# nv-tlabs/ChronoEdit

Hardware: AMD Instinct MI355X
Metric: denoising-steps/sec (higher is better)
Workload: dtype bf16

## Files before the change

chronoedit_amd/csrc/ce_attn.hip:

```cpp
#include <cstdlib>

#include "ce_common.h"

namespace {

constexpr int HD = 128;
constexpr int QW = 32;
constexpr int KVB = 64;
constexpr int K_TILE_BYTES = KVB * HD * 2;
constexpr int VT_TILE_BYTES = HD * KVB * 2;
constexpr int BUF_BYTES = K_TILE_BYTES + VT_TILE_BYTES;
constexpr int OST_ROW = HD * 2 + 16;
constexpr int smem_bytes(int nwave, bool two_seg) {
  const int stage = nwave * QW * OST_ROW;
  return two_seg ? 2 * BUF_BYTES + stage : (stage > 2 * BUF_BYTES ? stage : 2 * BUF_BYTES);
}
constexpr float NEG_BIG = -1.0e30f;

__device__ __forceinline__ int vt_swz(int dv) {
  return ((((dv >> 2) & 7) << 1) | (((dv >> 1) ^ (dv >> 5)) & 1)) ^ (((dv >> 6) & 1) << 1);
}

struct KVSeg {
  const bf16* k;
// ... 223 lines not shown
#pragma unroll
  for (int i = 0; i < 8; ++i) {
    const int c = lane + 64 * i;
    const int rl = c >> 4, cc = c & 15;
    const int q = q0 + rl;
    if (q < Nq) {
      const u32x4 v = *reinterpret_cast<const u32x4*>(smem + (TWO_SEG ? 2 * BUF_BYTES : 0) + (size_t)(wave * QW + rl) * OST_ROW + cc * 16);
      *reinterpret_cast<u32x4*>(O + (size_t)q * ldo + hoff + cc * 8) = v;
    }
  }
}


#define CE_EPOCH_BARRIER()                          \
  asm volatile("s_waitcnt lgkmcnt(0)" ::: "memory"); \
  __builtin_amdgcn_s_barrier()
constexpr int PK_ROW = HD * 2 + 16;
constexpr int PV_ROW = KVB * 2 + 16;
constexpr int PK_TILE = KVB * PK_ROW;
constexpr int PV_TILE = HD * PV_ROW;
typedef __attribute__((ext_vector_type(4))) unsigned pp_u4;
typedef __attribute__((ext_vector_type(2))) unsigned pp_u2;

constexpr int K_GRP = 1088;
typedef __attribute__((address_space(3))) void lds_void;
#ifdef CE_DIAGNOSTICS
__device__ unsigned long long g_sp_exact_hits = 0ull;
#endif
constexpr float SP_SPEC_THR = 1024.0f;
constexpr int SP_V0 = 2 * PK_TILE;
constexpr int SP_TILE_BYTES = 2 * PK_TILE + 3 * PV_TILE;
constexpr int sp_smem_bytes(bool two_seg) { return two_seg ? SP_TILE_BYTES + 8 * QW * OST_ROW : SP_TILE_BYTES; }

template <bool TWO_SEG, bool VT = false, bool QOUT = false>
__global__ __launch_bounds__(512, 2) void attn_fwd_sp_kernel(const bf16* __restrict__ Q_, bf16* __restrict__ O_, KVSeg seg0_,
                                                              KVSeg seg1_, int Nq, int H, int ldq, int ldo, int nqb,
                                                              float scale_log2e, int batch, BlkRows blk) {
  extern __shared__ __attribute__((aligned(16))) unsigned char smem[];
  constexpr int NWAVE = 8, QB = QW * NWAVE;
  const int tid = threadIdx.x, lane = tid & 63;
  const int wave = __builtin_amdgcn_readfirstlane(tid >> 6);
  const int l31 = lane & 31, hh = lane >> 5;
  for (int item = blockIdx.x; item < nqb * H * batch; item += gridDim.x) {
  const bf16* Q = Q_;
  bf16* O = O_;
  KVSeg seg0 = seg0_, seg1 = seg1_;

  int head, qb, bz;
  {
    const int nqb_full = Nq / QB;
    if ((H & 7) == 0) {
      const int xcd = item & 7, local = item >> 3, hx_n = H >> 3;
      const int full = batch * hx_n * nqb_full;
      if (local < full) {
        bz = local / (hx_n * nqb_full);
        const int r = local % (hx_n * nqb_full);
        head = xcd + 8 * (r / nqb_full);
        qb = r % nqb_full;
      } else {
        const int l2 = local - full;
        bz = l2 / hx_n;
        head = xcd + 8 * (l2 % hx_n);
        qb = nqb_full;
      }
    } else {
      bz = item / (nqb * H);
      const int r = item % (nqb * H);
      head = r / nqb;
      qb = r % nqb;
    }
  }
  {
    if (VT && blk.rows > 0) {
      Q += (size_t)bz * blk.rows * ldq;
      O += (size_t)bz * blk.rows * ldo;
      seg0.k += (size_t)bz * blk.rows * seg0.ldk;
      seg0.v += (size_t)bz * blk.vt_cols;
    } else {
      Q += (size_t)bz * Nq * ldq;
      O += (size_t)bz * Nq * ldo;
      seg0.k += (size_t)bz * seg0.len * seg0.ldk;
      seg0.v += VT ? (size_t)bz * (TWO_SEG ? blk.vt_cols : seg0.len) : (size_t)bz * seg0.len * seg0.ldv;
    }
    if (TWO_SEG) {
      seg1.k += (size_t)bz * seg1.len * seg1.ldk;
      seg1.v += VT ? (size_t)bz * blk.stride : (size_t)bz * seg1.len * seg1.ldv;
    }
  }
  const int q0 = qb * QB + wave * QW;
  const int hoff = head * HD;
  const bool active = q0 < Nq;
  const int q0row = (VT && blk.rows > 0) ? (q0 / blk.rows) * blk.stride + q0 % blk.rows : q0;

  bf16x8 qf[8];
  {
    const bf16* qrow = Q + (size_t)(q0 + l31 < Nq ? q0row + l31 : 0) * ldq + hoff + 8 * hh;
#pragma unroll
    for (int ks = 0; ks < 8; ++ks) qf[ks] = *reinterpret_cast<const bf16x8*>(qrow + 16 * ks);
  }
  auto scale_q = [&]() __attribute__((always_inline)) {
#pragma unroll
  for (int ks = 0; ks < 8; ++ks) {
    const u32x4 w = __builtin_bit_cast(u32x4, qf[ks]);
    u32x4 o;
#pragma unroll
    for (int i = 0; i < 4; ++i) o[i] = pack_bf16(bf16lo(w[i]) * scale_log2e, bf16hi(w[i]) * scale_log2e);
    qf[ks] = __builtin_bit_cast(bf16x8, o);
  }
#pragma unroll
  for (int ks = 0; ks < 8; ++ks) asm volatile("" : "+v"(qf[ks]));

  };
  const int v_dvq = (tid & 1) | (((tid >> 4) & 15) << 1), v_kvq = ((tid >> 1) & 7) | (((tid >> 8) & 1) << 3);
  const int v_chunk = (v_kvq & ~3) | ((v_kvq & 1) << 1) | ((v_kvq >> 1) & 1);
  unsigned char* ost = smem + (TWO_SEG ? SP_TILE_BYTES : 0) + (size_t)(wave * QW + l31) * OST_ROW;
  const int k_w = l31 & 3;
  const unsigned char* k_rd = smem + (l31 >> 2) * K_GRP + k_w * 256 + ((hh ^ (k_w & 1)) << 4);
  const int k_eo[2] = {(k_w >> 1) << 5, ((k_w >> 1) ^ 1) << 5};
  const unsigned char* v_rd = smem + SP_V0 + l31 * PV_ROW + hh * 16;
  int vt_off[4];
#pragma unroll
  for (int s4 = 0; s4 < 4; ++s4) {
    const int x = (l31 >> 1) & 7;
    vt_off[s4] = l31 * 128 + ((2 * (s4 ^ (x >> 1)) + (hh ^ (x & 1))) << 4);
  }
  unsigned char* v_wr = smem + SP_V0 + (4 * v_dvq) * PV_ROW + v_chunk * 8;

#pragma unroll
  for (int sidx = 0; sidx < (TWO_SEG ? 2 : 1); ++sidx) {
    const KVSeg sg = sidx == 0 ? seg0 : seg1;
    const int ntiles = (sg.len + KVB - 1) / KVB;
    const int k_rows_span = (VT && blk.rows > 0) ? ((sg.len - 1) / blk.rows) * blk.stride + blk.rows : sg.len;
    const auto k_rsrc = __builtin_amdgcn_make_buffer_rsrc((void*)(sg.k + hoff), 0, (k_rows_span - 1) * sg.ldk * 2 + HD * 2, 0x00020000);
    const auto v_rsrc = VT ? __builtin_amdgcn_make_buffer_rsrc((void*)(sg.v + (size_t)hoff * sg.ldv), 0, ((HD - 1) * sg.ldv + ntiles * KVB) * 2, 0x00020000)
                           : __builtin_amdgcn_make_buffer_rsrc((void*)(sg.v + hoff), 0, (sg.len - 1) * sg.ldv * 2 + HD * 2, 0x00020000);
    int v_voff[4];
#pragma unroll
    for (int i = 0; i < 4; ++i) v_voff[i] = (4 * v_kvq + i) * sg.ldv * 2 + v_dvq * 8;
    const int k_tile_bytes = KVB * sg.ldk * 2, v_tile_bytes = KVB * sg.ldv * 2;

    f32x16 oacc[4];
#pragma unroll
    for (int m = 0; m < 4; ++m)
#pragma unroll
      for (int r = 0; r < 16; ++r) oacc[m][r] = 0.f;
    float l_run = 0.f, alpha_prev = 1.0f, mc = 0.f;
    f32x16 cinit;
#pragma unroll
// ... 25 lines not shown
#pragma unroll
      for (int i = 0; i < 4; ++i) vreg[i] = __builtin_amdgcn_raw_buffer_load_b64(v_rsrc, v_voff[i], so, 0);
    };
    auto store_v_part = [&](int buf, int j) {
      const int w = j >> 1;
      uint32_t lo, hi;
      if ((j & 1) == 0) {
        lo = (vreg[0][w] & 0xffffu) | (vreg[1][w] << 16);
        hi = (vreg[2][w] & 0xffffu) | (vreg[3][w] << 16);
      } else {
        lo = (vreg[0][w] >> 16) | (vreg[1][w] & 0xffff0000u);
        hi = (vreg[2][w] >> 16) | (vreg[3][w] & 0xffff0000u);
      }
      pp_u2 val = {lo, hi};
      *reinterpret_cast<pp_u2*>(v_wr + buf * PV_TILE + j * PV_ROW) = val;
    };
    auto store_v = [&](int buf) {
#pragma unroll
      for (int j = 0; j < 4; ++j) {
        const int w = j >> 1;
        uint32_t lo, hi;
        if ((j & 1) == 0) {
          lo = (vreg[0][w] & 0xffffu) | (vreg[1][w] << 16);
          hi = (vreg[2][w] & 0xffffu) | (vreg[3][w] << 16);
        } else {
          lo = (vreg[0][w] >> 16) | (vreg[1][w] & 0xffff0000u);
          hi = (vreg[2][w] >> 16) | (vreg[3][w] & 0xffff0000u);
        }
        pp_u2 val = {lo, hi};
        *reinterpret_cast<pp_u2*>(v_wr + buf * PV_TILE + j * PV_ROW) = val;
      }
    };

    if (TWO_SEG && sidx == 1) { CE_EPOCH_BARRIER(); }
    dma_k(0, 0, 0);
    dma_k(0, 0, 1);
    __builtin_amdgcn_sched_barrier(0);
    if (VT) {
      dma_v(0, 0, 0);
      dma_v(0, 0, 1);
    } else {
      load_v(0);
    }
    {
      const pp_u4 z = {0u, 0u, 0u, 0u};
      for (int i = tid; i < PV_TILE / 16; i += NWAVE * 64) *reinterpret_cast<pp_u4*>(smem + SP_V0 + 2 * PV_TILE + i * 16) = z;
    }
    if (!VT) {
      store_v(0);
      asm volatile("s_waitcnt vmcnt(0)" ::: "memory");
      load_v(1);
    }
    if (sidx == 0) scale_q();

#define CE_SP_KWAIT()                                          \
  do {                                                         \
    if (VT) asm volatile("s_waitcnt vmcnt(2)" ::: "memory");   \
    else asm volatile("s_waitcnt vmcnt(4)" ::: "memory");      \
  } while (0)
    int vb_prev = 2, vb_cur = 0;

    for (int t = 0; !active && t < ntiles; ++t) {
      CE_SP_KWAIT();
      CE_EPOCH_BARRIER();
      const int vb_next = 3 - vb_prev - vb_cur;
      dma_k(t + 1, (t + 1) & 1, 0);
      dma_k(t + 1, (t + 1) & 1, 1);
      __builtin_amdgcn_sched_barrier(0);
      if (VT) {
        dma_v(t + 1, vb_next, 0);
        dma_v(t + 1, vb_next, 1);
      } else {
        store_v(vb_next);
        load_v(t + 2);
      }
      vb_prev = vb_cur;
      vb_cur = vb_next;
    }
    for (int t = 0; active && t < ntiles; ++t) {
      CE_SP_KWAIT();
      CE_EPOCH_BARRIER();
      const int vb_next = 3 - vb_prev - vb_cur;
      const unsigned char* kb = k_rd + (t & 1) * PK_TILE;
      const unsigned char* vb = v_rd + vb_prev * PV_TILE;
      const unsigned char* vtb = smem + SP_V0 + vb_prev * PV_TILE;

      const f32x16 zero16 = {0.f, 0.f, 0.f, 0.f, 0.f, 0.f, 0.f, 0.f, 0.f, 0.f, 0.f, 0.f, 0.f, 0.f, 0.f, 0.f};
      f32x16 st[2];
      {
        constexpr int RING = VT ? 4 : 6;
        bf16x8 kf[RING];
#define CE_LDK(i) (*reinterpret_cast<const bf16x8*>(kb + k_eo[((i) >> 1) & 1] + ((i) & 1) * 8 * K_GRP + ((i) >> 2) * 64))
#pragma unroll
// ... 107 lines not shown
          const bf16x8 kfr = *reinterpret_cast<const bf16x8*>(kb + k_eo[(i >> 1) & 1] + (i & 1) * 8 * K_GRP + (i >> 2) * 64);
          st[i & 1] = __builtin_amdgcn_mfma_f32_32x32x16_bf16(kfr, qf[i >> 1], i < 2 ? zero16 : st[i & 1], 0, 0, 0);
        }
#pragma unroll
        for (int f = 0; f < 2; ++f)
#pragma unroll
          for (int r = 0; r < 16; ++r) st[f][r] -= mc;
        mask_tail();
        rebase();
        psum = 0.f;
#pragma unroll
        for (int j = 0; j < 16; ++j) {
          st[j >> 3][(2 * j) & 15] = __builtin_amdgcn_exp2f(st[j >> 3][(2 * j) & 15]);
          st[j >> 3][(2 * j + 1) & 15] = __builtin_amdgcn_exp2f(st[j >> 3][(2 * j + 1) & 15]);
          psum += st[j >> 3][(2 * j) & 15] + st[j >> 3][(2 * j + 1) & 15];
          pack_pair(j);
        }
      }
      l_run = l_run * alpha + psum;
      alpha_prev = alpha;
      vb_prev = vb_cur;
      vb_cur = vb_next;
    }
    if (active && __any(alpha_prev != 1.0f)) {
#pragma unroll
      for (int m = 0; m < 4; ++m)
#pragma unroll
        for (int r = 0; r < 16; ++r) oacc[m][r] *= alpha_prev;
    }
    if (VT) {
      asm volatile("s_waitcnt vmcnt(0)" ::: "memory");
      __builtin_amdgcn_s_barrier();
    }
    if (active) {
      const unsigned char* vb = v_rd + vb_prev * PV_TILE;
      const unsigned char* vtb = smem + SP_V0 + vb_prev * PV_TILE;
#pragma unroll
      for (int u = 0; u < 16; ++u) {
        const bf16x8 vfd = VT ? *reinterpret_cast<const bf16x8*>(vtb + vt_off[u >> 2] + (u & 3) * 4096)
                              : *reinterpret_cast<const bf16x8*>(vb + (u & 3) * 32 * PV_ROW + (u >> 2) * 32);
        oacc[u & 3] = __builtin_amdgcn_mfma_f32_32x32x16_bf16(vfd, __builtin_bit_cast(bf16x8, ppk[u >> 2]), oacc[u & 3], 0, 0, 0);
      }
    }
    CE_EPOCH_BARRIER();

    const float l_tot = l_run + __shfl_xor(l_run, 32, 64);
    const float inv = 1.0f / l_tot;
#pragma unroll
    for (int m = 0; m < 4; ++m)
#pragma unroll
      for (int a = 0; a < 4; ++a) {
        uint32_t w0 = pack_bf16(oacc[m][4 * a + 0] * inv, oacc[m][4 * a + 1] * inv);
        uint32_t w1 = pack_bf16(oacc[m][4 * a + 2] * inv, oacc[m][4 * a + 3] * inv);
        u32x2* slot = reinterpret_cast<u32x2*>(ost + (32 * m + 8 * a + 4 * hh) * 2);
        if (TWO_SEG && sidx == 1) {
          const u32x2 pv = *slot;
          w0 = pack_bf16(bf16lo(pv[0]) + bf16lo(w0), bf16hi(pv[0]) + bf16hi(w0));
          w1 = pack_bf16(bf16lo(pv[1]) + bf16lo(w1), bf16hi(pv[1]) + bf16hi(w1));
        }
        u32x2 val = {w0, w1};
        *slot = val;
      }
  }

  if (TWO_SEG && VT && QOUT) {
    const int ktiles = (H * HD) >> 7;
    const int grow = bz * Nq + q0 + l31;
#pragma unroll
    for (int m = 0; m < 4; ++m) {
      uint32_t pk[8];
      float amax = 0.f;
#pragma unroll
      for (int a = 0; a < 4; ++a) {
        const u32x2 pv = *reinterpret_cast<const u32x2*>(ost + (32 * m + 8 * a + 4 * hh) * 2);
        pk[2 * a] = pv[0];
        pk[2 * a + 1] = pv[1];
        amax = fmaxf(amax, fmaxf(fmaxf(fabsf(bf16lo(pv[0])), fabsf(bf16hi(pv[0]))), fmaxf(fabsf(bf16lo(pv[1])), fabsf(bf16hi(pv[1])))));
      }
      amax = fmaxf(amax, __shfl_xor(amax, 32, 64));
      const int byte = mx_scale_byte_nosat(amax);
      const float is = mx_inv_scale(byte);
#pragma unroll
      for (int a = 0; a < 4; ++a) {
        int w = 0;
        w = __builtin_amdgcn_cvt_pk_fp8_f32(clamp448(bf16lo(pk[2 * a]) * is), clamp448(bf16hi(pk[2 * a]) * is), w, false);
        w = __builtin_amdgcn_cvt_pk_fp8_f32(clamp448(bf16lo(pk[2 * a + 1]) * is), clamp448(bf16hi(pk[2 * a + 1]) * is), w, true);
        *reinterpret_cast<uint32_t*>(ost + 32 * m + 8 * a + 4 * hh) = (uint32_t)w;
      }
      if (hh == 0 && q0 + l31 < Nq) blk.s8[mx_gemm_scale_offset(grow, head * 4 + m, ktiles)] = (unsigned char)byte;
    }
    __syncthreads();
    unsigned char* O8 = blk.q8 + (size_t)bz * Nq * blk.ld8;
#pragma unroll
    for (int i = 0; i < 4; ++i) {
      const int c = lane + 64 * i;
      const int rl = c >> 3, cc = c & 7;
      if (q0 + rl < Nq) {
        const u32x4 v = *reinterpret_cast<const u32x4*>(smem + SP_TILE_BYTES + (size_t)(wave * QW + rl) * OST_ROW + cc * 16);
        *reinterpret_cast<u32x4*>(O8 + (size_t)(q0 + rl) * blk.ld8 + hoff + cc * 16) = v;
      }
    }
  } else {
  __syncthreads();
#pragma unroll
  for (int i = 0; i < 8; ++i) {
    const int c = lane + 64 * i;
    const int rl = c >> 4, cc = c & 15;
    if (q0 + rl < Nq) {
      const u32x4 v = *reinterpret_cast<const u32x4*>(smem + (TWO_SEG ? SP_TILE_BYTES : 0) + (size_t)(wave * QW + rl) * OST_ROW + cc * 16);
      *reinterpret_cast<u32x4*>(O + (size_t)(q0row + rl) * ldo + hoff + cc * 8) = v;
    }
  }
  }
  __syncthreads();
  }
}


#define W4A_S_FIRST(ST, KF, QF, CI) asm volatile("v_mfma_f32_32x32x16_bf16 %0, %1, %2, %3" : "=&v"(ST) : "v"(KF), "a"(QF), "v"(CI))
#define W4A_S(ST, KF, QF) asm volatile("v_mfma_f32_32x32x16_bf16 %0, %1, %2, %0" : "+v"(ST) : "v"(KF), "a"(QF))
#define W4A_PV(OA, VF, PP) asm volatile("v_mfma_f32_32x32x16_bf16 %0, %1, %2, %0" : "+a"(OA) : "v"(VF), "v"(PP))
#define W4A_ADD(ACC, X) asm volatile("v_add_f32 %0, %0, %1" : "+v"(ACC) : "v"(X))
#define W4A_CVT(DST, A, B)                                                                  \
  do {                                                                                      \
    uint32_t w_;                                                                            \
    asm volatile("v_cvt_pk_bf16_f32 %0, %1, %2" : "=v"(w_) : "v"(A), "v"(B));               \
    (DST) = w_;                                                                             \
  } while (0)
#ifndef W4_KDMA_IN_PV
#define W4_KDMA_IN_PV 1
#endif
#ifndef W4_ABLATE
#define W4_ABLATE 0
#endif
#ifndef W4_EXP_ASM
#define W4_EXP_ASM 1
#endif
#if W4_EXP_ASM
#define W4A_EXP(X) asm volatile("v_exp_f32 %0, %0" : "+v"(X))
#else
#define W4A_EXP(X) (X) = __builtin_amdgcn_exp2f(X)
#endif
#define W4A_SETTLE_S(SB) asm volatile("s_nop 11" : "+v"(st[SB][0]), "+v"(st[SB][1]))
#define W4A_SETTLE_O(SB) asm volatile("s_nop 11" : "+a"(oacc[SB][0]), "+a"(oacc[SB][1]), "+a"(oacc[SB][2]), "+a"(oacc[SB][3]))
constexpr int W4_KB = 4;
constexpr int W4_V0 = W4_KB * PK_TILE;
constexpr int W4_SMEM = W4_V0 + 3 * PV_TILE;
// ... 445 lines not shown
      *reinterpret_cast<pp_u2*>(tile + (d0 + j) * TROW + kq * 8) = pp_u2{lo, hi};
    }
  }
  __syncthreads();
#pragma unroll
  for (int i = 0; i < 4; ++i) {
    const int c = tid + 256 * i;
    const int d = c >> 3, ch = c & 7;
    const pp_u4 v = *reinterpret_cast<const pp_u4*>(tile + d * TROW + ch * 16);
    const int col = key0 + 8 * ch;
    if (col < col_end) *reinterpret_cast<pp_u4*>(VT + (size_t)(head * HD + d) * ldvt + col) = v;
  }
}

}

#ifdef CE_DIAGNOSTICS
extern "C" int ce_diag_mx_exact_hits(unsigned long long* out, int reset);
CE_API int ce_diag_attention_exact_route_hits(unsigned long long* hits, int reset) {
  if (!hits) return CE_ERR_ARG;
  unsigned long long v = 0ull, z = 0ull;
  if (hipDeviceSynchronize() != hipSuccess) return CE_ERR_ARG;
  if (hipMemcpyFromSymbol(&v, HIP_SYMBOL(g_sp_exact_hits), sizeof(v)) != hipSuccess) return CE_ERR_ARG;
  if (reset && hipMemcpyToSymbol(HIP_SYMBOL(g_sp_exact_hits), &z, sizeof(z)) != hipSuccess) return CE_ERR_ARG;
  hits[0] = v;
  return ce_diag_mx_exact_hits(hits + 1, reset);
}
#endif
CE_KNOB g_attn_nwave = 0;
#ifdef CE_DIAGNOSTICS
CE_API int ce_set_attention_waves(int nwave) {
  const int old = g_attn_nwave;
  if (nwave == 0 || nwave == 4 || nwave == 8 || nwave == 16 || nwave == 64 || nwave == 128 || nwave == 129) g_attn_nwave = nwave;
  return old;
}
#endif

CE_API int ce_attention_batched_bf16(const void* Q, const void* K1, const void* V1, int len1, int ldk1, int ldv1,
                                         const void* K2, const void* V2, int len2, int ldk2, int ldv2, void* O, int Nq, int H,
                                         int head_dim, int ldq, int ldo, float softmax_scale, int batch, hipStream_t stream) {
  if (!Q || !K1 || !V1 || !O) return CE_ERR_ARG;
  if (head_dim != HD || Nq <= 0 || H <= 0 || len1 <= 0 || batch <= 0 || batch > 65535) return CE_ERR_SHAPE;
  if ((ldq & 7) || (ldo & 7) || (ldk1 & 7) || (ldv1 & 3)) return CE_ERR_ALIGN;
  const bool two = (K2 != nullptr && V2 != nullptr && len2 > 0);
  if (two && ((ldk2 & 7) || (ldv2 & 3))) return CE_ERR_ALIGN;
  KVSeg s0{(const bf16*)K1, (const bf16*)V1, len1, ldk1, ldv1};
  KVSeg s1{(const bf16*)K2, (const bf16*)V2, two ? len2 : 0, ldk2, ldv2};
  const float sl2 = softmax_scale * 1.4426950408889634f;
  const bool sp = g_attn_nwave == 64 || g_attn_nwave == 0 || g_attn_nwave >= 128;
  const int nwave = sp ? 8 : g_attn_nwave;
  const int nqb = (Nq + nwave * QW - 1) / (nwave * QW);
  dim3 grid(nqb * H, batch), block(nwave * 64);
  if (sp) {
#define CE_ATTN_SP(TWO)                                                                                              \
  do {                                                                                                               \
    static bool done_[CE_MAX_DEVICES] = {};                                                                          \
    bool& done = done_[ce_device_slot()];                                                                            \
    if (!done) {                                                                                                     \
      (void)hipFuncSetAttribute((const void*)attn_fwd_sp_kernel<TWO>, hipFuncAttributeMaxDynamicSharedMemorySize,    \
                                sp_smem_bytes(TWO));                                                                 \
      done = true;                                                                                                   \
    }                                                                                                                \
    hipLaunchKernelGGL((attn_fwd_sp_kernel<TWO>), dim3(nqb * H * batch), block, sp_smem_bytes(TWO), stream, (const bf16*)Q, \
                       (bf16*)O, s0, s1, Nq, H, ldq, ldo, nqb, sl2, batch, BlkRows{0, 0, 0u, 0});                    \
  } while (0)
    if (two) CE_ATTN_SP(true); else CE_ATTN_SP(false);
// ... 50 lines not shown

#ifdef CE_DIAGNOSTICS
extern "C" int ce_attn16_launch(const void* Q, const void* K, const void* Vt, int len, int ldk, int ldvt, void* O, int Nq, int H, int ldq, int ldo,
                                float sl2, int batch, int cus, hipStream_t stream);
#endif

static int attention_vt_launch(const void* Q, const void* K, const void* Vt, int len, int ldk, int ldvt, void* O, int Nq, int H, int head_dim,
                               int ldq, int ldo, float softmax_scale, int batch, int blk_rows, int blk_stride, int vt_sample_cols,
                               hipStream_t stream) {
  if (!Q || !K || !Vt || !O) return CE_ERR_ARG;
  if (head_dim != HD || Nq <= 0 || H <= 0 || len <= 0 || batch <= 0 || batch > 65535) return CE_ERR_SHAPE;
  const int ntiles_cols = (len + KVB - 1) / KVB * KVB;
  if (blk_rows == 0) {
    vt_sample_cols = len;
    if (ldvt < (batch - 1) * len + ntiles_cols) return CE_ERR_SHAPE;
  } else {
    if ((blk_rows & 63) || blk_stride < batch * blk_rows || (Nq % blk_rows) || vt_sample_cols < ntiles_cols ||
        ldvt < (batch - 1) * vt_sample_cols + ntiles_cols)
      return CE_ERR_SHAPE;
  }
  if ((ldq & 7) || (ldo & 7) || (ldk & 7) || (ldvt & 7) || (batch > 1 && (vt_sample_cols & 1))) return CE_ERR_ALIGN;
  KVSeg s0{(const bf16*)K, (const bf16*)Vt, len, ldk, ldvt};
  KVSeg s1{nullptr, nullptr, 0, 0, 0};
  BlkRows blk{blk_rows, blk_stride, 0u, vt_sample_cols};
  if (blk_rows > 0) {
    const uint32_t tps = (uint32_t)(blk_rows >> 6);
    blk.magic = tps == 1 ? 0u : (uint32_t)(((1ull << 32) + tps - 1) / tps);
  }
  const float sl2 = softmax_scale * 1.4426950408889634f;
  const int nqb = (Nq + 8 * QW - 1) / (8 * QW);
  static bool done_[CE_MAX_DEVICES] = {};
  bool& done = done_[ce_device_slot()];
  if (!done) {
    (void)hipFuncSetAttribute((const void*)attn_fwd_sp_kernel<false, true>, hipFuncAttributeMaxDynamicSharedMemorySize, sp_smem_bytes(false));
    done = true;
  }
  const int cus = ce_device_cus();
  const int items = nqb * H * batch;
#ifdef CE_DIAGNOSTICS
  if (g_attn_nwave == 16 && blk_rows == 0) {
    const int rc = ce_attn16_launch(Q, K, Vt, len, ldk, ldvt, O, Nq, H, ldq, ldo, sl2, batch, cus, stream);
    if (rc != CE_ERR_ALIGN) return rc;
  }
#endif
  if (g_attn_nwave == 128 || g_attn_nwave == 129) {
    static bool done4_[CE_MAX_DEVICES] = {};
    bool& done4 = done4_[ce_device_slot()];
    if (!done4) {
      (void)hipFuncSetAttribute((const void*)attn_fwd_w4_kernel, hipFuncAttributeMaxDynamicSharedMemorySize, W4_SMEM);
      done4 = true;
    }
    const int grid4 = (g_attn_nwave == 129 && items > cus) ? (cus & ~7) : items;
    hipLaunchKernelGGL(attn_fwd_w4_kernel, dim3(grid4), dim3(256), W4_SMEM, stream, (const bf16*)Q, (bf16*)O, s0, Nq, H, ldq, ldo, nqb,
                       sl2, batch, blk);
    return (int)hipGetLastError();
  }
  const int grid_vt = items <= 2 * cus ? items : ((2 * cus) & ~7);
  hipLaunchKernelGGL((attn_fwd_sp_kernel<false, true>), dim3(grid_vt), dim3(512), sp_smem_bytes(false), stream, (const bf16*)Q, (bf16*)O,
                     s0, s1, Nq, H, ldq, ldo, nqb, sl2, batch, blk);
  return (int)hipGetLastError();
}

CE_API int ce_attention_vt_bf16(const void* Q, const void* K, const void* Vt, int len, int ldk, int ldvt, void* O, int Nq, int H,
                                    int head_dim, int ldq, int ldo, float softmax_scale, int batch, hipStream_t stream) {
  return attention_vt_launch(Q, K, Vt, len, ldk, ldvt, O, Nq, H, head_dim, ldq, ldo, softmax_scale, batch, 0, 0, 0, stream);
}

CE_API int ce_attention_vt_blocked_bf16(const void* Q, const void* K, const void* Vt, int len, int ldk, int ldvt, void* O, int Nq, int H,
                                            int head_dim, int ldq, int ldo, float softmax_scale, int batch, int blk_rows, int blk_stride,
                                            int vt_sample_cols, hipStream_t stream) {
  if (blk_rows <= 0) return CE_ERR_SHAPE;
  return attention_vt_launch(Q, K, Vt, len, ldk, ldvt, O, Nq, H, head_dim, ldq, ldo, softmax_scale, batch, blk_rows, blk_stride, vt_sample_cols,
                             stream);
}


static int attention_2seg_vt_launch(const void* Q, const void* K1, const void* V1t, int len1, int ldk1, int ldv1t, int vt_cols1,
                                    const void* K2, const void* V2t, int len2, int ldk2, int ldv2t, int vt_cols2, void* O, int Nq,
                                    int H, int head_dim, int ldq, int ldo, float softmax_scale, int batch, void* O8, void* S8, int ldo8,
                                    hipStream_t stream) {
  if (!Q || !K1 || !V1t || !K2 || !V2t || (!O && !O8)) return CE_ERR_ARG;
  if (head_dim != HD || Nq <= 0 || H <= 0 || len1 <= 0 || len2 <= 0 || batch <= 0 || batch > 65535) return CE_ERR_SHAPE;
  const int c1 = (len1 + KVB - 1) / KVB * KVB, c2 = (len2 + KVB - 1) / KVB * KVB;
  if (vt_cols1 < len1 || vt_cols2 < len2 || ldv1t < (batch - 1) * vt_cols1 + c1 || ldv2t < (batch - 1) * vt_cols2 + c2) return CE_ERR_SHAPE;
  if ((ldq & 7) || (ldo & 7) || (ldk1 & 7) || (ldk2 & 7) || (ldv1t & 7) || (ldv2t & 7) || (vt_cols1 & 1) || (vt_cols2 & 1)) return CE_ERR_ALIGN;
  KVSeg s0{(const bf16*)K1, (const bf16*)V1t, len1, ldk1, ldv1t};
  KVSeg s1{(const bf16*)K2, (const bf16*)V2t, len2, ldk2, ldv2t};
  const float sl2 = softmax_scale * 1.4426950408889634f;
  const int nqb = (Nq + 8 * QW - 1) / (8 * QW);
  static bool done_[CE_MAX_DEVICES] = {};
  bool& done = done_[ce_device_slot()];
  if (!done) {
    (void)hipFuncSetAttribute((const void*)attn_fwd_sp_kernel<true, true>, hipFuncAttributeMaxDynamicSharedMemorySize, sp_smem_bytes(true));
    (void)hipFuncSetAttribute((const void*)attn_fwd_sp_kernel<true, true, true>, hipFuncAttributeMaxDynamicSharedMemorySize, sp_smem_bytes(true));
    done = true;
  }
  const BlkRows blk{0, vt_cols2, 0u, vt_cols1, (unsigned char*)O8, (unsigned char*)S8, ldo8};
  const int cus = ce_device_cus();
  const int items = nqb * H * batch;
  const int grid = items <= 2 * cus ? items : ((2 * cus) & ~7);
  if (O8)
    hipLaunchKernelGGL((attn_fwd_sp_kernel<true, true, true>), dim3(grid), dim3(512), sp_smem_bytes(true), stream, (const bf16*)Q,
                       (bf16*)O, s0, s1, Nq, H, ldq, ldo, nqb, sl2, batch, blk);
  else
    hipLaunchKernelGGL((attn_fwd_sp_kernel<true, true>), dim3(grid), dim3(512), sp_smem_bytes(true), stream, (const bf16*)Q, (bf16*)O,
                       s0, s1, Nq, H, ldq, ldo, nqb, sl2, batch, blk);
  return (int)hipGetLastError();
}

CE_API int ce_attention_2seg_vt_bf16(const void* Q, const void* K1, const void* V1t, int len1, int ldk1, int ldv1t, int vt_cols1,
                                         const void* K2, const void* V2t, int len2, int ldk2, int ldv2t, int vt_cols2, void* O, int Nq,
                                         int H, int head_dim, int ldq, int ldo, float softmax_scale, int batch, hipStream_t stream) {
  if (!O) return CE_ERR_ARG;
  return attention_2seg_vt_launch(Q, K1, V1t, len1, ldk1, ldv1t, vt_cols1, K2, V2t, len2, ldk2, ldv2t, vt_cols2, O, Nq, H, head_dim, ldq, ldo,
                                  softmax_scale, batch, nullptr, nullptr, 0, stream);
}

CE_API int ce_attention_2seg_vt_quant_bf16(const void* Q, const void* K1, const void* V1t, int len1, int ldk1, int ldv1t, int vt_cols1,
                                               const void* K2, const void* V2t, int len2, int ldk2, int ldv2t, int vt_cols2, void* o8,
                                               void* scale8, int Nq, int H, int head_dim, int ldq, int ldo8, float softmax_scale, int batch,
                                               hipStream_t stream) {
  if (!o8 || !scale8 || (ldo8 & 15) || ((H * head_dim) & 127)) return CE_ERR_ARG;
  return attention_2seg_vt_launch(Q, K1, V1t, len1, ldk1, ldv1t, vt_cols1, K2, V2t, len2, ldk2, ldv2t, vt_cols2, nullptr, Nq, H, head_dim, ldq,
                                  8, softmax_scale, batch, o8, scale8, ldo8, stream);
}
```

chronoedit_amd/hiplib.py:

```python
from __future__ import annotations

import ctypes
import os
import re
import subprocess
from typing import Dict, List

PKG_DIR = os.path.dirname(os.path.abspath(__file__))
ROOT = os.path.dirname(PKG_DIR)
CSRC = os.path.join(PKG_DIR, "csrc")
LIB_DIR = os.path.join(PKG_DIR, "lib")
LIB_PATH = os.path.join(LIB_DIR, "libchronoedit_hip.so")
DIAG_LIB_PATH = os.path.join(LIB_DIR, "libchronoedit_hip_diag.so")
OBJ_DIR = os.path.join(LIB_DIR, "obj")
HEADER = os.path.join(ROOT, "include", "chronoedit_hip.h")
DIAG_HEADER = os.path.join(ROOT, "include", "chronoedit_hip_diag.h")

DIAG_SOURCES = ["ce_gemm.hip", "ce_gemm256.hip", "ce_attn.hip", "ce_attn_fp8.hip", "ce_gemm_fp8.hip", "ce_gemm_fp8w4.hip"]
DIAG_ONLY_SOURCES = ["ce_attn16.hip"]
SOURCES = ["ce_rowops.hip", "ce_gemm.hip", "ce_gemm256.hip", "ce_gemm256w4.hip", "ce_gemm384.hip", "ce_attn.hip", "ce_attn16.hip", "ce_attn_fp8.hip", "ce_sched.hip", "ce_conv.hip", "ce_enc.hip", "ce_gemm_fp8.hip", "ce_gemm_fp8w4.hip", "ce_comm.hip"]

_c = ctypes
_P, _I, _F = _c.c_void_p, _c.c_int, _c.c_float

# ... 27 lines not shown
    "ce_gather_rows_bf16": [_P, _P, _P, _I, _I, _I, _I, _I, _P],
    "ce_rmsnorm_bf16": [_P, _P, _P, _I, _I, _I, _I, _F, _P],
    "ce_softmax_t5_bf16": [_P, _P, _I, _I, _I, _I, _I, _I, _P, _P, _P, _P],
    "ce_attention_bf16": [_P, _P, _P, _I, _I, _I, _P, _P, _I, _I, _I, _P, _I, _I, _I, _I, _I, _F, _P],
    "ce_attention_batched_bf16": [_P, _P, _P, _I, _I, _I, _P, _P, _I, _I, _I, _P, _I, _I, _I, _I, _I, _F, _I, _P],
    "ce_attention_vt_bf16": [_P, _P, _P, _I, _I, _I, _P, _I, _I, _I, _I, _I, _F, _I, _P],
    "ce_attention_2seg_vt_bf16": [_P, _P, _P, _I, _I, _I, _I, _P, _P, _I, _I, _I, _I, _P, _I, _I, _I, _I, _I, _F, _I, _P],
    "ce_attention_2seg_vt_quant_bf16": [_P, _P, _P, _I, _I, _I, _I, _P, _P, _I, _I, _I, _I, _P, _P, _I, _I, _I, _I, _I, _F, _I, _P],
    "ce_v_transpose_bf16": [_P, _I, _P, _I, _I, _I, _P],
    "ce_attention_vt_blocked_bf16": [_P, _P, _P, _I, _I, _I, _P, _I, _I, _I, _I, _I, _F, _I, _I, _I, _I, _P],
    "ce_v_transpose_blocked_bf16": [_P, _I, _P, _I, _I, _I, _I, _I, _I, _I, _P],
    "ce_timestep_sinusoid": [_P, _P, _I, _P],
    "ce_timestep_sinusoid_f32": [_P, _P, _I, _P],
    "ce_gemv": [_P, _I, _P, _P, _P, _I, _I, _I, _P],
    "ce_modulation": [_P, _P, _P, _I, _I, _I, _I, _I, _P],
    "ce_patchify_bf16": [_P, _P, _I, _I, _I, _I, _I, _P],
    "ce_unpatchify_bf16": [_P, _P, _I, _I, _I, _I, _I, _P],
    "ce_conv_igemm_bf16": [_P, _I, _P, _P, _P, _I, _P] + [_I] * 16 + [_P],
    "ce_conv3d_head_bf16": [_P, _I, _P, _P, _P, _I] + [_I] * 10 + [_P],
    "ce_gemm_bf16_tile_rows": [_I, _I, _I, _I, _c.c_longlong],
    "ce_zero_border_bf16": [_P, _I, _I, _I, _I, _I, _P],
    "ce_conv3d_gemm_bf16": [_P, _P, _I, _P, _P, _P, _I, _I, _I, _I, _I, _I, _I, _I, _P],
    "ce_conv3d_gemm_rms_silu_bf16": [_P, _P, _I, _P, _P, _P, _P, _I, _I, _I, _I, _I, _I, _I, _P, _I, _P],
    "ce_rms_silu_bf16": [_P, _P, _P, _c.c_longlong, _I, _I, _I, _I, _I, _I, _P],
    "ce_upsample2x_bf16": [_P, _P, _I, _I, _I, _I, _P],
    "ce_softmax_rows_f32_bf16": [_P, _P, _I, _I, _I, _I, _I, _F, _P],
    "ce_attention_1head_bf16": [_P, _P, _P, _P, _I, _I, _I, _I, _I, _I, _I, _F, _P, _c.c_longlong, _P],
    "ce_cfg_unipc_step": [_P, _P, _P, _P, _P, _P, _P, _P, _P, _c.c_longlong, _I, _P],
    "ce_build_info": [],
}
DIAG_SIGNATURES: Dict[str, List] = {
    "ce_set_gemm_variant": [_I],
    "ce_set_attention_waves": [_I],
    "ce_set_gemm_fp8_variant": [_I],
    "ce_set_attention_mxfp8_variant": [_I],
    "ce_set_attention_mxfp8_persistent": [_I],
    "ce_diag_attention_exact_route_hits": [_P, _I],
}


def header_symbols(diag: bool = False) -> List[str]:
    txt = open(DIAG_HEADER if diag else HEADER).read()
    return re.findall(r"^int (ce_\w+)\(", txt, flags=re.M)


def exported_symbols(path: str) -> List[str]:
    nm = "/opt/rocm/lib/llvm/bin/llvm-nm" if os.path.exists("/opt/rocm/lib/llvm/bin/llvm-nm") else "nm"
    out = subprocess.run([nm, "-D", "--defined-only", path], check=True, capture_output=True, text=True).stdout
    return sorted(l.split()[-1] for l in out.splitlines() if l.split() and l.split()[-2] in ("T", "t", "W", "D", "B"))


HIPCC_FLAGS = ["--offload-arch=gfx950", "-O3", "-std=c++17", "-fPIC", "-fvisibility=hidden"]


def build(force: bool = False, verbose: bool = False, jobs: int = 0) -> str:
    import glob
    from concurrent.futures import ThreadPoolExecutor
    srcs = [s for s in SOURCES if os.path.exists(os.path.join(CSRC, s))]
    hdrs = sorted(glob.glob(os.path.join(CSRC, "*.h"))) + [HEADER, DIAG_HEADER]
    hdr_m = max(os.path.getmtime(d) for d in hdrs)
    os.makedirs(OBJ_DIR, exist_ok=True)
    hipcc = os.environ.get("HIPCC", "/opt/rocm/bin/hipcc")
    todo, objs, diag_objs = [], [], []
    for s_ in srcs:
        src, stem = os.path.join(CSRC, s_), s_[:-4]
        variants = [("", [])] + ([(".diag", ["-DCE_DIAGNOSTICS"])] if s_ in DIAG_SOURCES else [])
# ... 83 lines not shown
```

chronoedit_amd/ops.py:

```python
from __future__ import annotations

import ctypes
from typing import Optional

import torch

from . import hiplib

EPI_BIAS, EPI_BIAS_GELU, EPI_GATE_RES, EPI_BIAS_GELU_ERF = 0, 1, 2, 3
EPI_F32, EPI_MUL, EPI_BIAS_ROW, EPI_BIAS_T = 4, 5, 6, 7

_lib = None
_product = None

_KNOB_DEFAULTS = {"ce_set_gemm_variant": -1, "ce_set_attention_waves": 0, "ce_set_gemm_fp8_variant": 1,
                  "ce_set_attention_mxfp8_variant": 1, "ce_set_attention_mxfp8_persistent": 512}
_knobs = dict(_KNOB_DEFAULTS)


def lib():
    global _lib, _product
    if _lib is None:
        _lib = _product = hiplib.load()
        import os
        v8 = os.environ.get("CE_GEMM_FP8_VARIANT")
        if v8 is not None:
            _set_knob("ce_set_gemm_fp8_variant", int(v8))
        v = os.environ.get("CE_GEMM_VARIANT")
        if v is not None:
            _set_knob("ce_set_gemm_variant", int(v))
    return _lib


_force_diag = False


def force_diagnostics(on: bool = True) -> None:
    global _lib, _force_diag
    lib()
    _force_diag = bool(on)
    want = hiplib.load_diagnostics() if (_force_diag or any(_knobs[k] != _KNOB_DEFAULTS[k] for k in _knobs)) else _product
    if want is not _lib:
        _lib = want


def attention_exact_route_hits(reset: bool = True):
    buf = (ctypes.c_ulonglong * 2)()
    _check(hiplib.load_diagnostics().ce_diag_attention_exact_route_hits(buf, 1 if reset else 0), "ce_diag_attention_exact_route_hits")
# ... 205 lines not shown
        buf = first[1]
    elif (dev, stream) in _gemm_own:
        buf = _gemm_own[(dev, stream)] = _gemm_own.pop((dev, stream))
    else:
        with torch.cuda.device(dev):
            capturing = torch.cuda.is_current_stream_capturing()
        if capturing:
            if first is None:
                return None, 0
            buf = first[1]
        elif first is None:
            buf = torch.empty(GEMM_WS_BYTES, dtype=torch.uint8, device=dev)
            _gemm_default[dev] = (stream, buf)
        else:
            mine = [k for k in _gemm_own if k[0] == dev]
            if len(mine) >= GEMM_WS_STREAMS:
                del _gemm_own[mine[0]]
            buf = _gemm_own[(dev, stream)] = torch.empty(GEMM_WS_BYTES, dtype=torch.uint8, device=dev)
    return buf.data_ptr(), buf.numel()


def set_gemm_split(on: bool) -> bool:
    global _gemm_split
    prev, _gemm_split = _gemm_split, bool(on)
    return prev


def set_gemm_variant(v: int) -> int:
    return _set_knob("ce_set_gemm_variant", v)


def set_attention_waves(n: int) -> int:
    return _set_knob("ce_set_attention_waves", n)


def attention(q: torch.Tensor, k: torch.Tensor, v: torch.Tensor, heads: int, out: Optional[torch.Tensor] = None,
              k2: Optional[torch.Tensor] = None, v2: Optional[torch.Tensor] = None, scale: Optional[float] = None,
              batch: int = 1):
    for n, t in (("q", q), ("k", k), ("v", v)):
        _dev(t, torch.bfloat16, n)
    Nq, Dq, ldq = _rows(q, "q")
    head_dim = Dq // heads
    L1, _, ldk = _rows(k, "k")
    L1v, _, ldv = _rows(v, "v")
    assert L1 == L1v
    if batch < 1 or Nq % batch or L1 % batch or (k2 is not None and k2.shape[0] % batch):
        raise ValueError(f"attention: row counts must be multiples of batch={batch}")
    if out is None:
        out = torch.empty((Nq, Dq), dtype=torch.bfloat16, device=q.device)
    _, _, ldo = _rows(out, "out")
    L2 = ldk2 = ldv2 = 0
    if k2 is not None:
        _dev(k2, torch.bfloat16, "k2"), _dev(v2, torch.bfloat16, "v2")
        L2, _, ldk2 = _rows(k2, "k2")
        _, _, ldv2 = _rows(v2, "v2")
    if scale is None:
        scale = head_dim ** -0.5
    st = _prof_begin()
    nq, l1, l2 = Nq // batch, L1 // batch, L2 // batch
    _check(lib().ce_attention_batched_bf16(_ptr(q), _ptr(k), _ptr(v), l1, ldk, ldv, _ptr(k2), _ptr(v2), l2, ldk2, ldv2, _ptr(out),
                                           nq, heads, head_dim, ldq, ldo, float(scale), batch, _stream()), "ce_attention_bf16")
    _prof_end(st, f"attention_{nq}x{l1}+{l2}_h{heads}" + (f"_b{batch}" if batch > 1 else ""),
              4.0 * nq * (l1 + l2) * head_dim * heads * batch)
    return out


# ... 675 lines not shown
```

include/chronoedit_hip_diag.h:

```cpp
#ifndef CHRONOEDIT_HIP_DIAG_H
#define CHRONOEDIT_HIP_DIAG_H

#include "chronoedit_hip.h"

#ifdef __cplusplus
extern "C" {
#endif

int ce_set_gemm_variant(int variant);

int ce_set_attention_waves(int nwave);

int ce_set_gemm_fp8_variant(int variant);

int ce_set_attention_mxfp8_variant(int variant);

int ce_set_attention_mxfp8_persistent(int n);

int ce_diag_attention_exact_route_hits(unsigned long long* hits, int reset);

#ifdef __cplusplus
}
#endif
#endif
```

Measured before the change: 2.973.

## Prefetch next work item's Q and first KV tile during attention epilogue

Adds an OVL template mode to the persistent attention kernel. Before the epilogue of the current item, it computes the next item's location, loads its Q, and issues LDS-DMA for its first K and V^T tiles (or the second segment's first tile). This hides the per-item pipeline fill latency behind the output store. The output staging area moves to a separate LDS region, and the trailing block-wide syncs become epoch barriers, which raises LDS use for the single-segment path and adds register pressure.

```diff
diff --git a/chronoedit_amd/csrc/ce_attn.hip b/chronoedit_amd/csrc/ce_attn.hip
--- a/chronoedit_amd/csrc/ce_attn.hip
+++ b/chronoedit_amd/csrc/ce_attn.hip
@@ -279,7 +279,15 @@
 constexpr int SP_TILE_BYTES = 2 * PK_TILE + 3 * PV_TILE;
 constexpr int sp_smem_bytes(bool two_seg) { return two_seg ? SP_TILE_BYTES + 8 * QW * OST_ROW : SP_TILE_BYTES; }
 
-template <bool TWO_SEG, bool VT = false, bool QOUT = false>
+struct SpItem {
+  const bf16* Q;
+  bf16* O;
+  KVSeg s0, s1;
+  int head, bz, q0, q0row, hoff;
+  bool active;
+};
+
+template <bool TWO_SEG, bool VT = false, bool QOUT = false, bool OVL = false>
 __global__ __launch_bounds__(512, 2) void attn_fwd_sp_kernel(const bf16* __restrict__ Q_, bf16* __restrict__ O_, KVSeg seg0_,
                                                               KVSeg seg1_, int Nq, int H, int ldq, int ldo, int nqb,
                                                               float scale_log2e, int batch, BlkRows blk) {
@@ -288,7 +296,11 @@
   const int tid = threadIdx.x, lane = tid & 63;
   const int wave = __builtin_amdgcn_readfirstlane(tid >> 6);
   const int l31 = lane & 31, hh = lane >> 5;
-  for (int item = blockIdx.x; item < nqb * H * batch; item += gridDim.x) {
+  static_assert(!OVL || VT, "the item overlap is built on the LDS-DMA staging of the V^T forms");
+  constexpr int OST0 = (TWO_SEG || OVL) ? SP_TILE_BYTES : 0;
+  const int n_items = nqb * H * batch;
+  auto locate = [&](int item) __attribute__((always_inline)) {
+  SpItem w;
   const bf16* Q = Q_;
   bf16* O = O_;
   KVSeg seg0 = seg0_, seg1 = seg1_;
@@ -335,16 +347,52 @@
     }
   }
   const int q0 = qb * QB + wave * QW;
-  const int hoff = head * HD;
-  const bool active = q0 < Nq;
-  const int q0row = (VT && blk.rows > 0) ? (q0 / blk.rows) * blk.stride + q0 % blk.rows : q0;
-
+  w.Q = Q;
+  w.O = O;
+  w.s0 = seg0;
+  w.s1 = seg1;
+  w.head = head;
+  w.bz = bz;
+  w.q0 = q0;
+  w.hoff = head * HD;
+  w.active = q0 < Nq;
+  w.q0row = (VT && blk.rows > 0) ? (q0 / blk.rows) * blk.stride + q0 % blk.rows : q0;
+  return w;
+  };
   bf16x8 qf[8];
-  {
-    const bf16* qrow = Q + (size_t)(q0 + l31 < Nq ? q0row + l31 : 0) * ldq + hoff + 8 * hh;
+  auto load_q = [&](const SpItem& w) __attribute__((always_inline)) {
+    const bf16* qrow = w.Q + (size_t)(w.q0 + l31 < Nq ? w.q0row + l31 : 0) * ldq + w.hoff + 8 * hh;
 #pragma unroll
     for (int ks = 0; ks < 8; ++ks) qf[ks] = *reinterpret_cast<const bf16x8*>(qrow + 16 * ks);
-  }
+  };
+  auto first_tile = [&](const KVSeg& s, int hoff_, int vbuf, int zbuf) __attribute__((always_inline)) {
+    const int nt = (s.len + KVB - 1) / KVB;
+    const int span = blk.rows > 0 ? ((s.len - 1) / blk.rows) * blk.stride + blk.rows : s.len;
+    const auto kr = __builtin_amdgcn_make_buffer_rsrc((void*)(s.k + hoff_), 0, (span - 1) * s.ldk * 2 + HD * 2, 0x00020000);
+    const auto vr = __builtin_amdgcn_make_buffer_rsrc((void*)(s.v + (size_t)hoff_ * s.ldv), 0, ((HD - 1) * s.ldv + nt * KVB) * 2, 0x00020000);
+    const int kdr = (lane >> 4) + 4 * ((wave >> 1) & 1) + 8 * (wave & 1) + 16 * (wave >> 2);
+    const int kd0 = kdr * s.ldk * 2 + (((lane & 15) ^ (lane >> 4)) << 4);
+    const int vdr = 8 * wave + (lane >> 3);
+    const int vd0 = vdr * s.ldv * 2 + (((lane & 7) ^ ((vdr >> 1) & 7)) << 4);
+    __builtin_amdgcn_raw_ptr_buffer_load_lds(kr, (lds_void*)(smem + wave * K_GRP), 16, kd0, 0, 0, 0);
+    __builtin_amdgcn_raw_ptr_buffer_load_lds(kr, (lds_void*)(smem + (wave + 8) * K_GRP), 16, kd0 + 32 * s.ldk * 2, 0, 0, 0);
+    __builtin_amdgcn_sched_barrier(0);
+    __builtin_amdgcn_raw_ptr_buffer_load_lds(vr, (lds_void*)(smem + SP_V0 + vbuf * PV_TILE + wave * 1024), 16, vd0, 0, 0, 0);
+    __builtin_amdgcn_raw_ptr_buffer_load_lds(vr, (lds_void*)(smem + SP_V0 + vbuf * PV_TILE + (wave + 8) * 1024), 16, vd0 + 64 * s.ldv * 2, 0, 0, 0);
+    const pp_u4 z = {0u, 0u, 0u, 0u};
+    for (int i = tid; i < PV_TILE / 16; i += NWAVE * 64) *reinterpret_cast<pp_u4*>(smem + SP_V0 + zbuf * PV_TILE + i * 16) = z;
+  };
+  bool pre = false;
+  int pre_v0 = 0, pre_z = 2;
+  SpItem nxt;
+  for (int item = blockIdx.x; item < n_items; item += gridDim.x) {
+  const SpItem it = (OVL && pre) ? nxt : locate(item);
+  const bf16* Q = it.Q;
+  bf16* O = it.O;
+  const KVSeg seg0 = it.s0, seg1 = it.s1;
+  const int head = it.head, bz = it.bz, q0 = it.q0, q0row = it.q0row, hoff = it.hoff;
+  const bool active = it.active;
+  if (!(OVL && pre)) load_q(it);
   auto scale_q = [&]() __attribute__((always_inline)) {
 #pragma unroll
   for (int ks = 0; ks < 8; ++ks) {
@@ -360,7 +408,7 @@
   };
   const int v_dvq = (tid & 1) | (((tid >> 4) & 15) << 1), v_kvq = ((tid >> 1) & 7) | (((tid >> 8) & 1) << 3);
   const int v_chunk = (v_kvq & ~3) | ((v_kvq & 1) << 1) | ((v_kvq >> 1) & 1);
-  unsigned char* ost = smem + (TWO_SEG ? SP_TILE_BYTES : 0) + (size_t)(wave * QW + l31) * OST_ROW;
+  unsigned char* ost = smem + OST0 + (size_t)(wave * QW + l31) * OST_ROW;
   const int k_w = l31 & 3;
   const unsigned char* k_rd = smem + (l31 >> 2) * K_GRP + k_w * 256 + ((hh ^ (k_w & 1)) << 4);
   const int k_eo[2] = {(k_w >> 1) << 5, ((k_w >> 1) ^ 1) << 5};
@@ -452,6 +500,7 @@
       }
     };
 
+    if (!(OVL && pre)) {
     if (TWO_SEG && sidx == 1) { CE_EPOCH_BARRIER(); }
     dma_k(0, 0, 0);
     dma_k(0, 0, 1);
@@ -466,6 +515,7 @@
       const pp_u4 z = {0u, 0u, 0u, 0u};
       for (int i = tid; i < PV_TILE / 16; i += NWAVE * 64) *reinterpret_cast<pp_u4*>(smem + SP_V0 + 2 * PV_TILE + i * 16) = z;
     }
+    }
     if (!VT) {
       store_v(0);
       asm volatile("s_waitcnt vmcnt(0)" ::: "memory");
@@ -478,7 +528,7 @@
     if (VT) asm volatile("s_waitcnt vmcnt(2)" ::: "memory");   \
     else asm volatile("s_waitcnt vmcnt(4)" ::: "memory");      \
   } while (0)
-    int vb_prev = 2, vb_cur = 0;
+    int vb_prev = (OVL && pre) ? pre_z : 2, vb_cur = (OVL && pre) ? pre_v0 : 0;
 
     for (int t = 0; !active && t < ntiles; ++t) {
       CE_SP_KWAIT();
@@ -652,6 +702,22 @@
       asm volatile("s_waitcnt vmcnt(0)" ::: "memory");
       __builtin_amdgcn_s_barrier();
     }
+    if (OVL) {
+      pre_v0 = vb_cur;
+      pre_z = 3 - vb_prev - vb_cur;
+      if (TWO_SEG && sidx == 0) {
+        first_tile(seg1, hoff, pre_v0, pre_z);
+        pre = true;
+      } else if (item + (int)gridDim.x < n_items) {
+        nxt = locate(item + gridDim.x);
+        load_q(nxt);
+        first_tile(nxt.s0, nxt.hoff, pre_v0, pre_z);
+        pre = true;
+      } else {
+        pre = false;
+      }
+      __builtin_amdgcn_sched_barrier(0);
+    }
     if (active) {
       const unsigned char* vb = v_rd + vb_prev * PV_TILE;
       const unsigned char* vtb = smem + SP_V0 + vb_prev * PV_TILE;
@@ -709,7 +775,7 @@
       }
       if (hh == 0 && q0 + l31 < Nq) blk.s8[mx_gemm_scale_offset(grow, head * 4 + m, ktiles)] = (unsigned char)byte;
     }
-    __syncthreads();
+    if (OVL) { CE_EPOCH_BARRIER(); } else { __syncthreads(); }
     unsigned char* O8 = blk.q8 + (size_t)bz * Nq * blk.ld8;
 #pragma unroll
     for (int i = 0; i < 4; ++i) {
@@ -721,18 +787,18 @@
       }
     }
   } else {
-  __syncthreads();
+  if (OVL) { CE_EPOCH_BARRIER(); } else { __syncthreads(); }
 #pragma unroll
   for (int i = 0; i < 8; ++i) {
     const int c = lane + 64 * i;
     const int rl = c >> 4, cc = c & 15;
     if (q0 + rl < Nq) {
-      const u32x4 v = *reinterpret_cast<const u32x4*>(smem + (TWO_SEG ? SP_TILE_BYTES : 0) + (size_t)(wave * QW + rl) * OST_ROW + cc * 16);
+      const u32x4 v = *reinterpret_cast<const u32x4*>(smem + OST0 + (size_t)(wave * QW + rl) * OST_ROW + cc * 16);
       *reinterpret_cast<u32x4*>(O + (size_t)(q0row + rl) * ldo + hoff + cc * 8) = v;
     }
   }
   }
-  __syncthreads();
+  if (!OVL) __syncthreads();
   }
 }
 
@@ -1244,6 +1310,15 @@
 CE_API int ce_set_attention_waves(int nwave) {
   const int old = g_attn_nwave;
   if (nwave == 0 || nwave == 4 || nwave == 8 || nwave == 16 || nwave == 64 || nwave == 128 || nwave == 129) g_attn_nwave = nwave;
+  return old;
+}
+#endif
+
+CE_KNOB g_attn_overlap = 1;
+#ifdef CE_DIAGNOSTICS
+CE_API int ce_set_attention_item_overlap(int on) {
+  const int old = g_attn_overlap;
+  if (on == 0 || on == 1) g_attn_overlap = on;
   return old;
 }
 #endif
@@ -1360,7 +1435,10 @@
   static bool done_[CE_MAX_DEVICES] = {};
   bool& done = done_[ce_device_slot()];
   if (!done) {
+    (void)hipFuncSetAttribute((const void*)attn_fwd_sp_kernel<false, true, false, true>, hipFuncAttributeMaxDynamicSharedMemorySize, sp_smem_bytes(true));
+#ifdef CE_DIAGNOSTICS
     (void)hipFuncSetAttribute((const void*)attn_fwd_sp_kernel<false, true>, hipFuncAttributeMaxDynamicSharedMemorySize, sp_smem_bytes(false));
+#endif
     done = true;
   }
   const int cus = ce_device_cus();
@@ -1384,8 +1462,15 @@
     return (int)hipGetLastError();
   }
   const int grid_vt = items <= 2 * cus ? items : ((2 * cus) & ~7);
-  hipLaunchKernelGGL((attn_fwd_sp_kernel<false, true>), dim3(grid_vt), dim3(512), sp_smem_bytes(false), stream, (const bf16*)Q, (bf16*)O,
-                     s0, s1, Nq, H, ldq, ldo, nqb, sl2, batch, blk);
+#ifdef CE_DIAGNOSTICS
+  if (!g_attn_overlap) {
+    hipLaunchKernelGGL((attn_fwd_sp_kernel<false, true>), dim3(grid_vt), dim3(512), sp_smem_bytes(false), stream, (const bf16*)Q, (bf16*)O,
+                       s0, s1, Nq, H, ldq, ldo, nqb, sl2, batch, blk);
+    return (int)hipGetLastError();
+  }
+#endif
+  hipLaunchKernelGGL((attn_fwd_sp_kernel<false, true, false, true>), dim3(grid_vt), dim3(512), sp_smem_bytes(true), stream, (const bf16*)Q,
+                     (bf16*)O, s0, s1, Nq, H, ldq, ldo, nqb, sl2, batch, blk);
   return (int)hipGetLastError();
 }
 
@@ -1419,20 +1504,35 @@
   static bool done_[CE_MAX_DEVICES] = {};
   bool& done = done_[ce_device_slot()];
   if (!done) {
+    (void)hipFuncSetAttribute((const void*)attn_fwd_sp_kernel<true, true, false, true>, hipFuncAttributeMaxDynamicSharedMemorySize, sp_smem_bytes(true));
+    (void)hipFuncSetAttribute((const void*)attn_fwd_sp_kernel<true, true, true, true>, hipFuncAttributeMaxDynamicSharedMemorySize, sp_smem_bytes(true));
+#ifdef CE_DIAGNOSTICS
     (void)hipFuncSetAttribute((const void*)attn_fwd_sp_kernel<true, true>, hipFuncAttributeMaxDynamicSharedMemorySize, sp_smem_bytes(true));
     (void)hipFuncSetAttribute((const void*)attn_fwd_sp_kernel<true, true, true>, hipFuncAttributeMaxDynamicSharedMemorySize, sp_smem_bytes(true));
+#endif
     done = true;
   }
   const BlkRows blk{0, vt_cols2, 0u, vt_cols1, (unsigned char*)O8, (unsigned char*)S8, ldo8};
   const int cus = ce_device_cus();
   const int items = nqb * H * batch;
   const int grid = items <= 2 * cus ? items : ((2 * cus) & ~7);
+#ifdef CE_DIAGNOSTICS
+  if (!g_attn_overlap) {
+    if (O8)
+      hipLaunchKernelGGL((attn_fwd_sp_kernel<true, true, true>), dim3(grid), dim3(512), sp_smem_bytes(true), stream, (const bf16*)Q,
+                         (bf16*)O, s0, s1, Nq, H, ldq, ldo, nqb, sl2, batch, blk);
+    else
+      hipLaunchKernelGGL((attn_fwd_sp_kernel<true, true>), dim3(grid), dim3(512), sp_smem_bytes(true), stream, (const bf16*)Q, (bf16*)O,
+                         s0, s1, Nq, H, ldq, ldo, nqb, sl2, batch, blk);
+    return (int)hipGetLastError();
+  }
+#endif
   if (O8)
-    hipLaunchKernelGGL((attn_fwd_sp_kernel<true, true, true>), dim3(grid), dim3(512), sp_smem_bytes(true), stream, (const bf16*)Q,
+    hipLaunchKernelGGL((attn_fwd_sp_kernel<true, true, true, true>), dim3(grid), dim3(512), sp_smem_bytes(true), stream, (const bf16*)Q,
                        (bf16*)O, s0, s1, Nq, H, ldq, ldo, nqb, sl2, batch, blk);
   else
-    hipLaunchKernelGGL((attn_fwd_sp_kernel<true, true>), dim3(grid), dim3(512), sp_smem_bytes(true), stream, (const bf16*)Q, (bf16*)O,
-                       s0, s1, Nq, H, ldq, ldo, nqb, sl2, batch, blk);
+    hipLaunchKernelGGL((attn_fwd_sp_kernel<true, true, false, true>), dim3(grid), dim3(512), sp_smem_bytes(true), stream, (const bf16*)Q,
+                       (bf16*)O, s0, s1, Nq, H, ldq, ldo, nqb, sl2, batch, blk);
   return (int)hipGetLastError();
 }
 
diff --git a/chronoedit_amd/hiplib.py b/chronoedit_amd/hiplib.py
--- a/chronoedit_amd/hiplib.py
+++ b/chronoedit_amd/hiplib.py
@@ -83,6 +83,7 @@
 DIAG_SIGNATURES: Dict[str, List] = {
     "ce_set_gemm_variant": [_I],
     "ce_set_attention_waves": [_I],
+    "ce_set_attention_item_overlap": [_I],
     "ce_set_gemm_fp8_variant": [_I],
     "ce_set_attention_mxfp8_variant": [_I],
     "ce_set_attention_mxfp8_persistent": [_I],
diff --git a/chronoedit_amd/ops.py b/chronoedit_amd/ops.py
--- a/chronoedit_amd/ops.py
+++ b/chronoedit_amd/ops.py
@@ -13,7 +13,7 @@
 _lib = None
 _product = None
 
-_KNOB_DEFAULTS = {"ce_set_gemm_variant": -1, "ce_set_attention_waves": 0, "ce_set_gemm_fp8_variant": 1,
+_KNOB_DEFAULTS = {"ce_set_gemm_variant": -1, "ce_set_attention_waves": 0, "ce_set_attention_item_overlap": 1, "ce_set_gemm_fp8_variant": 1,
                   "ce_set_attention_mxfp8_variant": 1, "ce_set_attention_mxfp8_persistent": 512}
 _knobs = dict(_KNOB_DEFAULTS)
 
@@ -285,6 +285,10 @@
 
 def set_attention_waves(n: int) -> int:
     return _set_knob("ce_set_attention_waves", n)
+
+
+def set_attention_item_overlap(on: bool) -> int:
+    return _set_knob("ce_set_attention_item_overlap", 1 if on else 0)
 
 
 def attention(q: torch.Tensor, k: torch.Tensor, v: torch.Tensor, heads: int, out: Optional[torch.Tensor] = None,
diff --git a/include/chronoedit_hip_diag.h b/include/chronoedit_hip_diag.h
--- a/include/chronoedit_hip_diag.h
+++ b/include/chronoedit_hip_diag.h
@@ -11,6 +11,8 @@
 
 int ce_set_attention_waves(int nwave);
 
+int ce_set_attention_item_overlap(int on);
+
 int ce_set_gemm_fp8_variant(int variant);
 
 int ce_set_attention_mxfp8_variant(int variant);
```

After: 2.968. No clear change (-0.2%).
